# JJKK1313/DiTreeOnlinePlanner

Hardware: AMD Instinct MI355X
Metric: candidate tree-expansions/sec (carmaze, H=32) (higher is better)
Workload: dtype f16x3; 1 GPU; cfgs/carmaze.yaml + fm_policy flow sampler (K=1), batch=1024 candidates per GPU, H=32 (4 chunks x 8 steps), boxes.csv 20x20, 1024-node tree snapshot, seeded random weights; batch_per_gpu=1024, global_batch=1024, edge_length=32, action_horizon=8, pred_horizon=64, flow_steps=1, tree_nodes=1024, parallelism=candidates sharded x1

## Files before the change

ditreeonlineplanner_amd/csrc/denoise.h:

```cpp
#pragma once
#include <hip/hip_runtime.h>
#include <stdint.h>

enum { MODE_BIAS = 0, MODE_GN_MISH = 1, MODE_GN_MISH_FILM = 2, MODE_GN_MISH_RES = 3 };

enum { ST_BF16 = 0, ST_F32 = 1, ST_F16 = 2 };
static inline int fmt_make(int st, bool split) { return st | (split ? 4 : 0); }
static inline __host__ __device__ int fmt_st(int f) { return f & 3; }
static inline __host__ __device__ bool fmt_split(int f) { return (f & 4) != 0; }
static inline int fmt_es(int f) { return fmt_st(f) == ST_F32 ? 4 : 2; }

struct ConvGemmParams {
  const void* A;
  int lda;
  int in_Lp;
  int in_stride;
  int in_off;
  int taps, Cin;
  const void* W;
  void* Out;
  int ldc;
  int out_Lp, out_stride, out_off;
  int out_coff;
  int L;
  int M, N;
  const float* bias;
  int mode;
  const float* gamma;
  const float* beta;
  int group_ch;
  float eps;
  const float* film;
  int film_ld, film_off;
  const void* Res;
  int ldres, res_Lp, res_off;
  int out_f32;
  int dbg;
  int c2d, c2_H, c2_W, c2_OW, c2_OHW, c2_stride, c2_pad;
  signed char c2_kh[12], c2_kw[12];
  const void* zero;
  long long a_plane, w_plane, out_plane, res_plane;
  float w_scale;
  int splitk;
  long long slab_stride;
  float* sk_ws;
  int* sk_cnt;
  int* sat;
};

void denoise_set_dry_run(bool on);
void launch_conv_gemm(const ConvGemmParams& p, int fmt, hipStream_t s);
bool conv2d_small_eligible(int fmt);
int conv_gemm_kind(const ConvGemmParams& p, int fmt);
bool conv_gemm_supported(const ConvGemmParams& p, int fmt);
void launch_prep_sample(const float* x, void* A0, int B, int P, int D, int fmt, long long plane, hipStream_t s, int* sat = nullptr);
void launch_time_embed(float t, const float* W1, const float* b1, const float* W2, const float* b2, float* out,
                       hipStream_t s);
void launch_prep_cond(const float* temb, const float* map_emb, int E, int E_ld, const float* cond, int G, void* out, int B,
                      int Kpad, int fmt, long long plane, hipStream_t s, int* sat = nullptr);
struct FlowStep {
  int mode;
  float dt;
  float sb, sa, c0, c1, sigma;
  const float* z;
  long long z_row;
  const int* z_idx;
  int z_row0;
};
void launch_final_proj_flow(const void* Y, int C, int Lp, long long plane, const float* W, const float* bias, int D, float* x,
                            FlowStep fs, const double* act_norm , double* actions, int B, int P, int fmt,
                            hipStream_t s);
struct TapList {
  int n;
  signed char kh[49], kw[49];
};
void launch_gn1d(void* x, int ld, int Lp, int row_off, int coff, int L, int C, const float* gamma, const float* beta, float eps,
                 int mode, const float* film, int film_ld, int film_off, const void* res, int ldres, int res_Lp, int res_off,
                 int B, int fmt, long long x_plane, long long res_plane, hipStream_t s, int* sat = nullptr);
void launch_encoder_stem(const float* lm, int n, const float* W, const float* gamma, const float* beta, void* out, int B, float eps,
                         int fmt, long long plane, hipStream_t s, int* sat = nullptr);
void launch_im2col2d(const void* in, bool src_f32, void* out, int B, int H, int W, int C, const TapList& taps, int stride,
                     int pad, int OH, int OW, int Kpad, int fmt, hipStream_t s);
void launch_gn2d(const float* in, int nslab, long long slab_stride, const float* gamma, const float* beta, const void* res,
                 int relu, void* out, int B, int HW, int C, float eps, int fmt, long long res_plane, long long out_plane,
                 hipStream_t s, int* sat = nullptr);
void launch_maxpool2d(const void* in, void* out, int B, int H, int W, int C, int OH, int OW, int fmt, hipStream_t s);
void launch_avgpool2d(const void* in, void* out, int B, int HW, int C, int fmt, long long in_plane, long long out_plane,
                      hipStream_t s);
void launch_unpack_act(const void* in, int ld, int coff, int Lp, int roff, float* out, int B, int L, int C, int fmt,
                       long long plane, hipStream_t s);
```

ditreeonlineplanner_amd/csrc/denoise_host.hip:

```cpp
#include <algorithm>
#include <cmath>
#include <cstring>
#include <functional>
#include <map>
#include <sstream>
#include <thread>

#include "denoise.h"
#include "ditree_internal.h"

namespace {

struct HostParam {
  std::vector<int64_t> dims;
  const float* data = nullptr;
  int64_t n = 0;
};

struct Act {
  void* p = nullptr;
  int L = 0, C = 0;
  int ld = 0, coff = 0;
  bool padded = true;
  long long plane = 0;
// ... 321 lines not shown
    p.Out = (void*)aptr(out); p.ldc = out.ld; p.out_Lp = out.Lp(); p.out_stride = 1; p.out_off = 1; p.out_coff = 0;
    p.L = in.L; p.N = Cout; p.bias = vec(wname + ".bias"); p.mode = mode; p.eps = 1e-5f;
    if (mode >= MODE_GN_MISH) {
      p.gamma = vec(gn + ".weight"); p.beta = vec(gn + ".bias"); p.group_ch = Cout / 8;
    }
    if (mode == MODE_GN_MISH_FILM) { p.film = film; p.film_ld = film_cols; p.film_off = film_off; }
    if (mode == MODE_GN_MISH_RES) {
      p.Res = aptr(*res); p.ldres = res->ld; p.res_Lp = res->Lp(); p.res_off = res->padded ? 1 : 0; p.res_plane = res->plane;
    }
    emit_block(ops, p, out, in.L);
  }
  void emit_block(std::vector<std::function<void(int, int, hipStream_t)>>& ops, const ConvGemmParams& p, const Act& out, int L) {
    const int Cout = p.N, mode = p.mode, uf = ufmt;
    const int gch = Cout / 8;
    static const bool short_unfused = [] { const char* e = getenv("DITREE_GN_SHORT_UNFUSED"); return e && atoi(e) != 0; }();
    const bool short_fusable = (L == 8 || L == 4) && fmt_st(uf) != ST_F32 && !short_unfused;
    const bool fused = mode < MODE_GN_MISH ||
                       ((Cout & 255) == 0 && (gch == 64 || gch == 128 || gch == 256) && ((L & 15) == 0 || short_fusable));
    const bool fused_needs_tiles = fused && mode >= MODE_GN_MISH && (L & 15) != 0;
    ConvGemmParams qf = p, q = p;
    q.mode = MODE_BIAS;
    const float* film_p = p.film;
    const int film_ld_ = p.film_ld, film_off_ = p.film_off, ldres = p.ldres, res_Lp = p.res_Lp, res_off = p.res_off;
    const void* resp = p.Res;
    const float *ga = p.gamma, *be = p.beta;
    void* xo = (void*)out.p;
    const int ld = out.ld, oLp = out.Lp(), ocoff = out.coff;
    const long long xpl = out.plane, rpl = p.res_plane;
    int* gsat = p.sat;
    ops.push_back([=, this](int, int Bp, hipStream_t s) mutable {
      if (fused && (!fused_needs_tiles || ((Bp * L) & 255) == 0)) {
        qf.M = Bp * L;
        run_gemm(qf, uf, s);
        return;
      }
      q.M = Bp * L;
      run_gemm(q, uf, s);
      note_other();
      launch_gn1d(xo, ld, oLp, 1, ocoff, L, Cout, ga, be, 1e-5f, mode, film_p, film_ld_, film_off_, resp, ldres, res_Lp,
                  res_off, Bp, uf, xpl, rpl, s, gsat);
    });
  }
  void add_conv1(std::vector<std::function<void(int, int, hipStream_t)>>& ops, const std::string& wname, const Act& in,
                 const Act& out) {
    const HostParam& w = P_(wname + ".weight");
    const int Cout = (int)w.dims[0], Cin = (int)w.dims[1];
    const float* wd = w.data;
    const Packed wp = pack(wname, ufmt, Cout, 1, Cin, [=](int n, int, int ci) { return wd[(size_t)n * Cin + ci]; });
    ConvGemmParams p{};
    p.A = aptr(in); p.lda = in.ld; p.in_Lp = in.Lp(); p.in_stride = 1; p.in_off = 1; p.taps = 1; p.Cin = Cin;
    set_w(p, wp); set_in(p, in); set_out(p, out);
    p.sat = sat_slot(wname, ufmt);
    p.Out = (void*)aptr(out); p.ldc = out.ld; p.out_Lp = out.Lp(); p.out_stride = 1; p.out_off = 1;
    p.L = in.L; p.N = Cout; p.bias = vec(wname + ".bias"); p.mode = MODE_BIAS;
    const int L = in.L, uf = ufmt;
    ops.push_back([this, p, L, uf](int, int Bp, hipStream_t s) mutable {
      p.M = Bp * L;
      run_gemm(p, uf, s);
    });
  }
  void add_down(std::vector<std::function<void(int, int, hipStream_t)>>& ops, const std::string& wname, const Act& in,
                const Act& out) {
    const HostParam& w = P_(wname + ".weight");
    const int Cout = (int)w.dims[0], Cin = (int)w.dims[1];
    const float* wd = w.data;
    const Packed wp = pack(wname, ufmt, Cout, 3, Cin, [=](int n, int t, int ci) { return wd[((size_t)n * Cin + ci) * 3 + t]; });
    ConvGemmParams p{};
    p.A = aptr(in); p.lda = in.ld; p.in_Lp = in.Lp(); p.in_stride = 2; p.in_off = 0; p.taps = 3; p.Cin = Cin;
    set_w(p, wp); set_in(p, in); set_out(p, out);
    p.sat = sat_slot(wname, ufmt);
    p.Out = (void*)aptr(out); p.ldc = out.ld; p.out_Lp = out.Lp(); p.out_stride = 1; p.out_off = 1;
    p.L = out.L; p.N = Cout; p.bias = vec(wname + ".bias"); p.mode = MODE_BIAS;
    const int L = out.L, uf = ufmt;
    ops.push_back([this, p, L, uf](int, int Bp, hipStream_t s) mutable {
      p.M = Bp * L;
      run_gemm(p, uf, s);
    });
  }
  void add_up(std::vector<std::function<void(int, int, hipStream_t)>>& ops, const std::string& wname, const Act& in,
              const Act& out) {
    const HostParam& w = P_(wname + ".weight");
    const int Cin = (int)w.dims[0], Cout = (int)w.dims[1];
    const float* wd = w.data;
    for (int par = 0; par < 2; ++par) {
      const int k0 = par == 0 ? 3 : 2, k1 = par == 0 ? 1 : 0;
      const Packed wp = pack(wname + (par ? ".odd" : ".even"), ufmt, Cout, 2, Cin, [=](int n, int t, int ci) {
        return wd[((size_t)ci * Cout + n) * 4 + (t == 0 ? k0 : k1)];
      });
      ConvGemmParams p{};
      p.A = aptr(in); p.lda = in.ld; p.in_Lp = in.Lp(); p.in_stride = 1; p.in_off = par; p.taps = 2; p.Cin = Cin;
      set_w(p, wp); set_in(p, in); set_out(p, out);
      p.sat = sat_slot(wname, ufmt);
      p.Out = (void*)aptr(out); p.ldc = out.ld; p.out_Lp = out.Lp(); p.out_stride = 2; p.out_off = 1 + par;
      p.L = in.L; p.N = Cout; p.bias = vec(wname + ".bias"); p.mode = MODE_BIAS;
      const int L = in.L, uf = ufmt;
      ops.push_back([this, p, L, uf](int, int Bp, hipStream_t s) mutable {
        p.M = Bp * L;
        run_gemm(p, uf, s);
      });
    }
  }

  void add_crb(const std::string& pre, const Act& in, const Act& out, int& film_cursor, const std::string& tag) {
    const int Cout = (int)P_(pre + ".blocks.0.block.0.weight").dims[0];
    Act h = make_act(tag + ".h", in.L, Cout);
    const int film_off = film_cursor;
    film_cursor += 2 * Cout;
    add_conv3(unet_ops, pre + ".blocks.0.block.0", in, h, MODE_GN_MISH_FILM, pre + ".blocks.0.block.1", film_off, nullptr);
    Act res = in;
    if (has(pre + ".residual_conv.weight")) {
      res = make_act(tag + ".res", in.L, Cout);
      add_conv1(unet_ops, pre + ".residual_conv", in, res);
    }
    add_conv3(unet_ops, pre + ".blocks.1.block.0", h, out, MODE_GN_MISH_RES, pre + ".blocks.1.block.1", 0, &res);
  }

  void build(int prec_, int Bmax_);
};

void DenoiserState::build(int prec_, int Bmax_) {
  free_workspace();
  prec = prec_;
  switch (prec) {
    case DITREE_PREC_BF16: ufmt = fmt_make(ST_BF16, false); efmt = ST_BF16; break;
    case DITREE_PREC_F32: ufmt = fmt_make(ST_F32, false); efmt = ST_F32; break;
    case DITREE_PREC_F16X3: ufmt = fmt_make(ST_F16, true); efmt = ufmt; break;
    case DITREE_PREC_BF16X3: ufmt = fmt_make(ST_BF16, true); efmt = ufmt; break;
    case DITREE_PREC_F16: ufmt = fmt_make(ST_F16, false); efmt = ST_F16; break;
    default: throw std::runtime_error("unknown precision");
  }
  sat_flags = (int*)dalloc(SAT_SLOTS * sizeof(int));
  sat_cond = sat_slot("cond_encoder input: Mish(time | map embedding | observation)", ufmt);
  sat_sample = sat_slot("sample (the noisy action sequence)", ufmt);
  const int C0 = dims[0], C1 = dims[1], C2 = dims[2];
  const int L0 = P, L1 = P / 2, L2 = P / 4;
  if (P % 16 != 0 || P < 16 || P > 256 || (256 % P) != 0) throw std::runtime_error("pred_horizon must be 16, 32, 64, 128 or 256");
  bgran = fmt_st(ufmt) != ST_F32 ? std::max(16, 1024 / P) : 16;
  Buser = Bmax_;
  Bmax = (Bmax_ + bgran - 1) / bgran * bgran;
  {
    const long long per_sample = std::max({(long long)(L2 + 2) * 2 * C2, (long long)(L1 + 2) * 2 * C1, (long long)(L0 + 2) * C0,
                                           (long long)L0 * 64}) * fmt_es(ufmt);
    long long cap = std::min<long long>(8192, 0x7f000000LL / per_sample);
    cap = cap / 256 * 256;
    if (cap < 256) throw std::runtime_error("denoiser too large for one 256-sample work unit");
    if (Bmax > cap) Bmax = (int)cap;
  }
  if (fmt_split(ufmt) && ((C0 | C1 | C2) & 255) != 0)
    throw std::runtime_error("the split precisions need down_dims that are multiples of 256 (halo / gemm16 tiles)");
  x_cur = (float*)dalloc((size_t)Bmax * P * D * 4);
  temb = (float*)dalloc(256 * 4);
  condK = (cond_dim + 63) / 64 * 64;
  const int Brows = (Bmax + 255) / 256 * 256;
  E_ld = fmt_split(efmt) ? (E + 255) / 256 * 256 : E;
  map_emb = (float*)dalloc((size_t)Brows * E_ld * 4);
  cond_plane = planes() == 2 ? (long long)Brows * condK * es() : 0;
  condA = dalloc((size_t)Brows * condK * es() * planes());

  std::vector<std::string> crbs = {"unet.down_modules.0.0", "unet.down_modules.0.1", "unet.down_modules.1.0",
                                   "unet.down_modules.1.1", "unet.down_modules.2.0", "unet.down_modules.2.1",
                                   "unet.mid_modules.0",    "unet.mid_modules.1",    "unet.up_modules.0.0",
                                   "unet.up_modules.0.1",   "unet.up_modules.1.0",   "unet.up_modules.1.1"};
  film_cols = 0;
  std::vector<int> film_offs;
  for (auto& c : crbs) {
    film_offs.push_back(film_cols);
// ... 782 lines not shown
```

ditreeonlineplanner_amd/csrc/denoise_kernels.hip:

```cpp
#include <cstdlib>
#include <type_traits>

#include <stdexcept>

#include "denoise.h"

static thread_local bool g_dn_dry_run = false;
void denoise_set_dry_run(bool on) { g_dn_dry_run = on; }
#define DN_LAUNCH(...) do { if (!g_dn_dry_run) hipLaunchKernelGGL(__VA_ARGS__); } while (0)

typedef __attribute__((ext_vector_type(8))) __bf16 bf16x8_t;
typedef __attribute__((ext_vector_type(8))) _Float16 half8_t;
typedef __attribute__((ext_vector_type(8))) short short8_t;
typedef __attribute__((ext_vector_type(4))) short short4_t;
typedef __attribute__((ext_vector_type(16))) float f32x16_t;
typedef __attribute__((ext_vector_type(4))) float f32x4_t;
typedef __attribute__((ext_vector_type(2))) float f32x2_t;
typedef __attribute__((ext_vector_type(2))) _Float16 half2_t;
typedef __attribute__((ext_vector_type(2))) short short2_t;

#define GLOBAL_AS __attribute__((address_space(1)))
#define LDS_AS __attribute__((address_space(3)))

__device__ __forceinline__ unsigned short f2bf(float f) {
// ... 450 lines not shown
#pragma unroll
      for (int i = 0; i < 16; ++i) acc[mb][j][i] = 0.0f;

  const int swl = (r5 >> 1) & 7;
  const int a_row_off = (wm * 64 + r5) * 128;
  const int b_row_off = 32768 + (wn * 128 + r5) * 128;

  auto kstep = [&](const char* sb, auto stage_tag, char* snext) {
    constexpr bool STAGE = decltype(stage_tag)::value;
    if constexpr (PREC != 1) {
      short8_t af[2][2], bfr[2][4];
      auto rd = [&](int ks, int slot) {
        const int ps = (((ks << 1) | h) ^ swl) << 4;
#pragma unroll
        for (int mb = 0; mb < 2; ++mb)
          af[slot][mb] = *(const short8_t*)(sb + a_row_off + mb * 4096 + ps);
#pragma unroll
        for (int j = 0; j < 4; ++j)
          bfr[slot][j] = *(const short8_t*)(sb + b_row_off + j * 4096 + ps);
      };
      if constexpr (STAGE) {
#pragma unroll
        for (int q = 0; q < 8; ++q) stage_piece(q, snext);
      }
      rd(0, 0);
#pragma unroll
      for (int ks = 0; ks < 4; ++ks) {
        if (ks < 3) rd(ks + 1, (ks + 1) & 1);
#pragma unroll
        for (int mb = 0; mb < 2; ++mb)
#pragma unroll
          for (int j = 0; j < 4; ++j)
            acc[mb][j] = mfma32<ET>(af[ks & 1][mb], bfr[ks & 1][j], acc[mb][j]);
      }
      if constexpr (STAGE) __builtin_amdgcn_sched_group_barrier(0x020, 8, 0);
      __builtin_amdgcn_sched_group_barrier(0x100, 6, 0);
#pragma unroll
      for (int ks = 0; ks < 4; ++ks) {
        if (ks < 3) __builtin_amdgcn_sched_group_barrier(0x100, 6, 0);
        __builtin_amdgcn_sched_group_barrier(0x008, 8, 0);
      }
    } else {
#pragma unroll
      for (int sl = 0; sl < 8; ++sl) {
        const int ps = (sl ^ swl) << 4;
        f32x4_t af[2], bfr[4];
#pragma unroll
        for (int mb = 0; mb < 2; ++mb) af[mb] = *(const f32x4_t*)(sb + a_row_off + mb * 4096 + ps);
#pragma unroll
        for (int j = 0; j < 4; ++j) bfr[j] = *(const f32x4_t*)(sb + b_row_off + j * 4096 + ps);
#pragma unroll
        for (int s2 = 0; s2 < 2; ++s2) {
#pragma unroll
          for (int mb = 0; mb < 2; ++mb) {
            const float a = h ? af[mb][2 * s2 + 1] : af[mb][2 * s2];
#pragma unroll
            for (int j = 0; j < 4; ++j) {
              const float bv = h ? bfr[j][2 * s2 + 1] : bfr[j][2 * s2];
              acc[mb][j] = __builtin_amdgcn_mfma_f32_32x32x2f32(a, bv, acc[mb][j], 0, 0, 0);
            }
          }
        }
        if constexpr (STAGE) stage_piece(sl, snext);
      }
    }
  };

#pragma unroll
  for (int q = 0; q < 8; ++q) stage_piece(q, smem);
  advance();
  for (int kt = 0; kt < nk - 1; ++kt) {
    asm volatile("s_waitcnt vmcnt(0)" ::: "memory");
    __syncthreads();
    kstep(smem + (kt & 1) * 65536, std::true_type{}, smem + ((kt + 1) & 1) * 65536);
    advance();
  }
  asm volatile("s_waitcnt vmcnt(0)" ::: "memory");
  __syncthreads();
  kstep(smem + ((nk - 1) & 1) * 65536, std::false_type{}, nullptr);
  __syncthreads();
  gemm_epilogue<PREC>(p, acc, smem, tm, tn, tid, lane, r5, h, wm, wn, out_extra);
}

template <int ET, bool SPLIT, bool SHORT = false>
__device__ __forceinline__ void gemm_epilogue16(const ConvGemmParams& p, f32x4_t (&acc)[4][8], char* smem, int tm, int tn,
                                                int tid, int lane, int r4, int h4, int wm, int wn) {
  const int c_l = wn * 128 + 8 * r4;
  const int n0 = tn * 256 + c_l;
  {
    f32x4_t b0 = {0.f, 0.f, 0.f, 0.f}, b1 = b0;
    if (p.bias != nullptr) { b0 = *(const f32x4_t*)(p.bias + n0); b1 = *(const f32x4_t*)(p.bias + n0 + 4); }
    if constexpr (ET == 1) {
      const float ws = p.w_scale;
#pragma unroll
      for (int mb = 0; mb < 4; ++mb)
#pragma unroll
        for (int j = 0; j < 4; ++j) { acc[mb][j] = acc[mb][j] * ws + b0[j]; acc[mb][4 + j] = acc[mb][4 + j] * ws + b1[j]; }
    } else if (p.bias != nullptr) {
#pragma unroll
      for (int mb = 0; mb < 4; ++mb)
#pragma unroll
        for (int j = 0; j < 4; ++j) { acc[mb][j] += b0[j]; acc[mb][4 + j] += b1[j]; }
    }
  }
  constexpr bool short_l = SHORT;
  const int lane_b = short_l ? (4 * h4) / p.L : 0, lane_l = -lane_b * p.L;
  int blk_b[4], blk_l[4];
#pragma unroll
  for (int mb = 0; mb < 4; ++mb) {
    const int m0 = tm * 256 + wm * 64 + mb * 16;
    const int b = m0 / p.L;
    blk_b[mb] = b;
    blk_l[mb] = m0 - b * p.L;
  }
  auto store_row = [&](char* o, const float (&v)[8]) {
    short8_t hi, lo;
    if constexpr (ET == 1) {
      sat_check_row(p.sat, v);
#pragma unroll
      for (int jj = 0; jj < 4; ++jj) {
        const f32x2_t c = {__builtin_amdgcn_fmed3f(v[2 * jj], -65504.0f, 65504.0f),
                           __builtin_amdgcn_fmed3f(v[2 * jj + 1], -65504.0f, 65504.0f)};
        const half2_t h = __builtin_convertvector(c, half2_t);
        const short2_t hs = __builtin_bit_cast(short2_t, h);
        hi[2 * jj] = hs[0]; hi[2 * jj + 1] = hs[1];
        if constexpr (SPLIT) {
          const half2_t l = __builtin_convertvector(c - __builtin_convertvector(h, f32x2_t), half2_t);
          const short2_t ls = __builtin_bit_cast(short2_t, l);
          lo[2 * jj] = ls[0]; lo[2 * jj + 1] = ls[1];
        }
      }
    } else {
#pragma unroll
      for (int j = 0; j < 8; ++j) {
        hi[j] = (short)f2bf(v[j]);
        if constexpr (SPLIT) lo[j] = (short)f2bf(v[j] - bf2f((unsigned short)hi[j]));
      }
    }
    *(short8_t*)o = hi;
    if constexpr (SPLIT) *(short8_t*)(o + p.out_plane) = lo;
  };
  auto out_ptr = [&](int mb, int esize) {
    const long long orow = (long long)(blk_b[mb] + lane_b) * p.out_Lp + (long long)(blk_l[mb] + 4 * h4 + lane_l) * p.out_stride + p.out_off;
    return (char*)p.Out + (orow * p.ldc + p.out_coff + n0) * esize;
  };
  if (p.mode < MODE_GN_MISH) {
    const int esize = p.out_f32 ? 4 : 2;
    const long long ostep = (long long)p.out_stride * p.ldc * esize;
#pragma unroll
    for (int mb = 0; mb < 4; ++mb) {
      char* ob = out_ptr(mb, esize);
#pragma unroll
      for (int i = 0; i < 4; ++i, ob += ostep) {
        float v[8];
#pragma unroll
        for (int j = 0; j < 8; ++j) v[j] = acc[mb][j][i];
        if (p.out_f32) {
          *(f32x4_t*)ob = f32x4_t{v[0], v[1], v[2], v[3]};
          *(f32x4_t*)(ob + 16) = f32x4_t{v[4], v[5], v[6], v[7]};
        } else {
          store_row(ob, v);
        }
      }
    }
    return;
  }
  const bool has_film = p.mode == MODE_GN_MISH_FILM, has_res = p.mode == MODE_GN_MISH_RES;
  const int spt = 256 / p.L;
  const int ns = spt > 16 ? spt * 4 : 64;
  float* s_sum = (float*)smem;
  float* s_sq = s_sum + ns;
  float* s_gb = s_sq + ns;
  float* s_film = s_gb + 512;
  const bool film_direct = has_film && short_l;
  const int b_last = p.M / p.L - 1;
  for (int i = tid; i < 2 * ns; i += 512) s_sum[i] = 0.0f;
  s_gb[tid] = tid < 256 ? p.gamma[tn * 256 + tid] : p.beta[tn * 256 + tid - 256];
  if (has_film && !film_direct) {
    for (int idx = tid; idx < spt * 128; idx += 512) {
      const int sm = idx >> 7, c4 = idx & 127;
      const int b = min(tm * spt + sm, b_last);
      const float* src = p.film + (long long)b * p.film_ld + p.film_off + tn * 256 + (c4 & 63) * 4 + (c4 >> 6) * p.N;
      *(f32x4_t*)(s_film + sm * 512 + c4 * 4) = *(const f32x4_t*)src;
    }
  }
  f32x4_t rh[2], rl[2];
  const long long rstep = (long long)p.ldres * 2;
  auto fetch_film = [&](int mb) {
    const float* fr = p.film + (long long)min(blk_b[mb] + lane_b, b_last) * p.film_ld + p.film_off + n0;
    rh[0] = *(const f32x4_t*)fr; rh[1] = *(const f32x4_t*)(fr + 4);
    rl[0] = *(const f32x4_t*)(fr + p.N); rl[1] = *(const f32x4_t*)(fr + p.N + 4);
  };
  if (film_direct) fetch_film(0);
  auto fetch_res = [&](int r) {
    const long long rrow = (long long)(blk_b[r >> 2] + lane_b) * p.res_Lp + blk_l[r >> 2] + 4 * h4 + lane_l + p.res_off;
    const char* rp = (const char*)p.Res + (rrow * p.ldres + n0) * 2 + (r & 3) * rstep;
    rh[r & 1] = *(const f32x4_t*)rp;
    if constexpr (SPLIT) rl[r & 1] = *(const f32x4_t*)(rp + p.res_plane);
  };
  if (has_res) { fetch_res(0); fetch_res(1); }
  __syncthreads();
  const int gi = c_l / p.group_ch;
  const bool wide = p.group_ch >= 128;
  const float inv_cnt = 1.0f / (float)(p.group_ch * p.L);
  int slot[4];
#pragma unroll
  for (int mb = 0; mb < 4; ++mb) slot[mb] = (blk_b[mb] + lane_b - tm * spt) * 4 + gi;
  const int hsame = short_l ? (p.L == 8 ? 2 : 1) : 4;
  const bool adder = (r4 == 0 || (!wide && r4 == 8)) && (h4 & (hsame - 1)) == 0;
  auto block_sums = [&](float (&s)[4], float* cell) {
#pragma unroll
    for (int mb = 0; mb < 4; ++mb) s[mb] = dpp_add<0xB1>(s[mb]);
#pragma unroll
    for (int mb = 0; mb < 4; ++mb) s[mb] = dpp_add<0x4E>(s[mb]);
#pragma unroll
    for (int mb = 0; mb < 4; ++mb) s[mb] = dpp_add<0x141>(s[mb]);
    if (wide) {
#pragma unroll
      for (int mb = 0; mb < 4; ++mb) s[mb] = dpp_add<0x140>(s[mb]);
    }
    if (hsame >= 2) {
#pragma unroll
      for (int mb = 0; mb < 4; ++mb) s[mb] += __shfl_xor(s[mb], 16);
    }
    if (hsame == 4) {
#pragma unroll
      for (int mb = 0; mb < 4; ++mb) s[mb] += __shfl_xor(s[mb], 32);
    }
    if (adder) {
#pragma unroll
      for (int mb = 0; mb < 4; ++mb) atomicAdd(&cell[slot[mb]], s[mb]);
    }
  };
  float mean_[4], rstd_[4];
  auto pair = [&](int mb, int j, int ip) { return f32x2_t{acc[mb][j][2 * ip], acc[mb][j][2 * ip + 1]}; };
  if constexpr (!SPLIT) {
    float s[4], q[4];
#pragma unroll
    for (int mb = 0; mb < 4; ++mb) {
      f32x2_t s2 = {0.f, 0.f}, q2 = {0.f, 0.f};
#pragma unroll
      for (int j = 0; j < 8; ++j)
#pragma unroll
        for (int ip = 0; ip < 2; ++ip) {
          const f32x2_t v = pair(mb, j, ip);
          s2 += v;
          q2 = __builtin_elementwise_fma(v, v, q2);
        }
      s[mb] = s2[0] + s2[1];
// ... 905 lines not shown
      mm16(0, 0, 0);
      __builtin_amdgcn_sched_group_barrier(0x100, 4, 0);
      __builtin_amdgcn_sched_group_barrier(0x008, 16, 0);
      __builtin_amdgcn_sched_barrier(0);
      mm16(1, 0, 0);
      __builtin_amdgcn_sched_barrier(0);
      mm16(0, 1, 1);
      __builtin_amdgcn_sched_barrier(0);
    } else {
      rdB(1, k, 0, 1);
      mm16(0, 0, 0);
      __builtin_amdgcn_sched_group_barrier(0x100, 4, 0);
      __builtin_amdgcn_sched_group_barrier(0x008, 16, 0);
      __builtin_amdgcn_sched_barrier(0);
      rdA(1, k, 1);
      rdB(0, k, 1, 0);
      mm16(0, 1, 1);
      __builtin_amdgcn_sched_group_barrier(0x100, 8, 0);
      __builtin_amdgcn_sched_group_barrier(0x008, 16, 0);
      __builtin_amdgcn_sched_barrier(0);
      rdB(1, k, 1, 1);
      mm16(1, 0, 0);
      __builtin_amdgcn_sched_group_barrier(0x100, 4, 0);
      __builtin_amdgcn_sched_group_barrier(0x008, 16, 0);
      __builtin_amdgcn_sched_barrier(0);
    }
    int ao2 = 0, wo2 = 0;
    if constexpr (ISSUE) src_off(k + 2, ao2, wo2);
    if constexpr (HAS_NEXT) {
      asm volatile("s_waitcnt vmcnt(0) lgkmcnt(0)" ::: "memory");
      __builtin_amdgcn_s_barrier();
      rdA(0, k + 1, 0);
      rdB(0, k + 1, SPLIT ? 1 : 0, 0);
    }
#pragma unroll
    for (int mb = 0; mb < 4; ++mb)
#pragma unroll
      for (int jj = 0; jj < 4; ++jj) {
        mm(1, 1, 1, mb, (mb & 1) ? 3 - jj : jj);
        if constexpr (ISSUE) {
          const int m = mb * 4 + jj, i = (m & 1) ? -1 : (m >> 1);
          if (i >= 0 && i < 4)
            __builtin_amdgcn_raw_ptr_buffer_load_lds(a_rsrc, (LDS_AS void*)(smem + (k & 1) * BUF + (w * 4 + i) * 1024), 16,
                                                     (i & 1) ? pao : pae, aq[i] + ao2, 0, 0);
          else if (!SPLIT && i >= 4 && i < 8)
            __builtin_amdgcn_raw_ptr_buffer_load_lds(w_rsrc, (LDS_AS void*)(smem + W_BASE + (k & 1) * BUF + (w * 4 + i - 4) * 1024),
                                                     16, ((i - 4) & 1) ? pbo : pbe, wq[i - 4] + wo2, 0, 0);
        }
      }
    if constexpr (HAS_NEXT) __builtin_amdgcn_sched_group_barrier(0x100, 8, 1);
#pragma unroll
    for (int i = 0; i < 16; ++i) {
      __builtin_amdgcn_sched_group_barrier(0x008, 1, 1);
      if (ISSUE && !(i & 1) && (!SPLIT || i < 8)) __builtin_amdgcn_sched_group_barrier(0x020, 1, 1);
    }
    __builtin_amdgcn_sched_barrier(0);
  };
  using Tt = std::true_type;
  using Ff = std::false_type;

  issue(0);
  asm volatile("s_waitcnt vmcnt(0)" ::: "memory");
  __builtin_amdgcn_s_barrier();
  if (nk > 1) {
    if constexpr (SPLIT) {
      int ao, wo;
      src_off(1, ao, wo);
#pragma unroll
      for (int q = 0; q < 4; ++q)
        __builtin_amdgcn_raw_ptr_buffer_load_lds(a_rsrc, (LDS_AS void*)(smem + BUF + (w * 4 + q) * 1024), 16, (q & 1) ? pao : pae,
                                                 aq[q] + ao, 0, 0);
    } else {
      issue(1);
    }
  }
  rdA(0, 0, 0);
  rdB(0, 0, SPLIT ? 1 : 0, 0);
  for (int k = 0; k < nk - 2; ++k) step(Tt{}, Tt{}, k);
  if (nk >= 2) step(Tt{}, Ff{}, nk - 2);
  step(Ff{}, Ff{}, nk - 1);
  __syncthreads();
  gemm_epilogue16<ET, SPLIT, SHORT>(p, acc, smem, tm, tn, tid, lane, r4, h4, wm, wn);
}
static bool gemm16_eligible(const ConvGemmParams& p, int fmt) {
  const bool short_ok = p.L == 8 || p.L == 4;
  return fmt_st(fmt) != ST_F32 && !p.c2d && (!p.out_f32 || p.mode == MODE_BIAS) && p.taps >= 1 && p.taps <= 3 && (p.M & 255) == 0 &&
         (p.N & 255) == 0 && (p.Cin & 63) == 0 && ((p.L & 15) == 0 || short_ok) && p.M > 0 &&
         (p.mode == MODE_BIAS || (256 % p.L) == 0);
}
static bool halo_eligible(const ConvGemmParams& p, int fmt) {
  static const bool l8_off = [] { const char* e = getenv("DITREE_HALO_L8"); return e && atoi(e) == 0; }();
  static const bool l4_off = [] { const char* e = getenv("DITREE_HALO_L4"); return e && atoi(e) == 0; }();
  const bool l_ok = p.L >= 16 || (p.L == 8 && fmt_split(fmt) && !l8_off) || (p.L == 4 && fmt_split(fmt) && !l4_off && p.splitk <= 1);
  return fmt_st(fmt) != ST_F32 && !p.c2d && p.taps == 3 && p.in_stride == 1 && p.in_Lp == p.L + 2 && (256 % p.L) == 0 &&
         l_ok && (p.M & 255) == 0 && (p.N & 255) == 0 && (p.Cin & 63) == 0 && p.Cin >= 192;
}
bool conv2d_small_eligible(int fmt) { return fmt_st(fmt) != ST_F32; }
int conv_gemm_kind(const ConvGemmParams& p, int fmt) { return halo_eligible(p, fmt) ? 0 : (p.c2d ? 2 : 1); }
bool conv_gemm_supported(const ConvGemmParams& p, int fmt) {
  return !fmt_split(fmt) || halo_eligible(p, fmt) || gemm16_eligible(p, fmt) ||
         (p.c2d && (p.N & 63) == 0 && (p.Cin & 63) == 0 && p.out_f32 && p.mode == MODE_BIAS);
}

static void ensure_lds_attrs() {
  static bool done[64] = {};
  int dev = 0;
  hipGetDevice(&dev);
  if (dev < 0 || dev >= 64 || done[dev]) return;
  done[dev] = true;
  const hipFuncAttribute at = hipFuncAttributeMaxDynamicSharedMemorySize;
  hipFuncSetAttribute((const void*)conv_gemm_kernel<0, false>, at, 131072);
  hipFuncSetAttribute((const void*)conv_gemm_kernel<1, false>, at, 131072);
  hipFuncSetAttribute((const void*)conv_gemm_kernel<2, false>, at, 131072);
  hipFuncSetAttribute((const void*)conv_gemm_kernel<0, true>, at, 131072);
  hipFuncSetAttribute((const void*)conv_gemm_kernel<1, true>, at, 131072);
  hipFuncSetAttribute((const void*)conv_gemm_kernel<2, true>, at, 131072);
  hipFuncSetAttribute((const void*)conv3_halo16_kernel<0, false>, at, 147456);
  hipFuncSetAttribute((const void*)conv3_halo16_kernel<1, false>, at, 147456);
  hipFuncSetAttribute((const void*)conv3_halo16x3_kernel<0>, at, 147456);
  hipFuncSetAttribute((const void*)conv3_halo16x3_kernel<1>, at, 147456);
  hipFuncSetAttribute((const void*)conv3_halo16x3_kernel<0, true>, at, 147456);
  hipFuncSetAttribute((const void*)conv3_halo16x3_kernel<1, true>, at, 147456);
  hipFuncSetAttribute((const void*)conv3_halo16x3_kernel<0, false, true>, at, 147456);
  hipFuncSetAttribute((const void*)conv3_halo16x3_kernel<1, false, true>, at, 147456);
  hipFuncSetAttribute((const void*)conv3_halo16x3_kernel<0, true, true>, at, 147456);
  hipFuncSetAttribute((const void*)conv3_halo16x3_kernel<1, true, true>, at, 147456);
  hipFuncSetAttribute((const void*)conv3_halo16x3_kernel<0, true, false, 6>, at, 163840);
  hipFuncSetAttribute((const void*)conv3_halo16x3_kernel<1, true, false, 6>, at, 163840);
  hipFuncSetAttribute((const void*)gemm16_kernel<0, false>, at, 131072);
  hipFuncSetAttribute((const void*)gemm16_kernel<1, false>, at, 131072);
  hipFuncSetAttribute((const void*)gemm16_kernel<0, true>, at, 131072);
  hipFuncSetAttribute((const void*)gemm16_kernel<1, true>, at, 131072);
  hipFuncSetAttribute((const void*)gemm16_kernel<0, false, true>, at, 131072);
  hipFuncSetAttribute((const void*)gemm16_kernel<1, false, true>, at, 131072);
  hipFuncSetAttribute((const void*)gemm16_kernel<0, true, true>, at, 131072);
  hipFuncSetAttribute((const void*)gemm16_kernel<1, true, true>, at, 131072);
}

void launch_conv_gemm(const ConvGemmParams& p, int fmt, hipStream_t s) {
  ensure_lds_attrs();
  const int st = fmt_st(fmt);
  const bool split = fmt_split(fmt), f16 = st == ST_F16;
  const int ntn = (p.N + 255) >> 8, ntm = (p.M + 255) >> 8;
  const dim3 grid(ntm * ntn), block(512);
  if (halo_eligible(p, fmt)) {
    if (split && p.splitk > 1) {
      if (p.sk_ws == nullptr || p.sk_cnt == nullptr || ((p.Cin >> 5) % p.splitk) != 0 || (p.Cin >> 5) / p.splitk < 2)
        throw std::runtime_error("conv_gemm: split-K of the halo kernel needs its workspace and splitk | Cin / 32, >= 2 chunks each");
      const dim3 gsk(ntm * ntn, p.splitk);
      if (p.L == 8) {
        if (f16) DN_LAUNCH((conv3_halo16x3_kernel<1, true, true>), gsk, block, 147456, s, p);
        else DN_LAUNCH((conv3_halo16x3_kernel<0, true, true>), gsk, block, 147456, s, p);
      } else if (f16) DN_LAUNCH((conv3_halo16x3_kernel<1, false, true>), gsk, block, 147456, s, p);
      else DN_LAUNCH((conv3_halo16x3_kernel<0, false, true>), gsk, block, 147456, s, p);
      return;
    }
    if (split && p.L == 4) {
      if (f16) DN_LAUNCH((conv3_halo16x3_kernel<1, true, false, 6>), grid, block, 163840, s, p);
      else DN_LAUNCH((conv3_halo16x3_kernel<0, true, false, 6>), grid, block, 163840, s, p);
      return;
    }
    if (split) {
      if (p.L == 8) {
        if (f16) DN_LAUNCH((conv3_halo16x3_kernel<1, true>), grid, block, 147456, s, p);
        else DN_LAUNCH((conv3_halo16x3_kernel<0, true>), grid, block, 147456, s, p);
      } else if (f16) DN_LAUNCH(conv3_halo16x3_kernel<1>, grid, block, 147456, s, p);
      else DN_LAUNCH(conv3_halo16x3_kernel<0>, grid, block, 147456, s, p);
    } else {
      if (f16) DN_LAUNCH((conv3_halo16_kernel<1, false>), grid, block, 147456, s, p);
      else DN_LAUNCH((conv3_halo16_kernel<0, false>), grid, block, 147456, s, p);
    }
    return;
  }
  if (gemm16_eligible(p, fmt) && (p.L & 15) != 0) {
    if (split) {
      if (f16) DN_LAUNCH((gemm16_kernel<1, true, true>), grid, block, 131072, s, p);
      else DN_LAUNCH((gemm16_kernel<0, true, true>), grid, block, 131072, s, p);
    } else {
      if (f16) DN_LAUNCH((gemm16_kernel<1, false, true>), grid, block, 131072, s, p);
      else DN_LAUNCH((gemm16_kernel<0, false, true>), grid, block, 131072, s, p);
    }
    return;
  }
  if (gemm16_eligible(p, fmt)) {
    if (split) {
      if (f16) DN_LAUNCH((gemm16_kernel<1, true>), grid, block, 131072, s, p);
      else DN_LAUNCH((gemm16_kernel<0, true>), grid, block, 131072, s, p);
    } else {
      if (f16) DN_LAUNCH((gemm16_kernel<1, false>), grid, block, 131072, s, p);
      else DN_LAUNCH((gemm16_kernel<0, false>), grid, block, 131072, s, p);
    }
    return;
  }
  if (p.mode >= MODE_GN_MISH && (p.L & 15) != 0)
    throw std::runtime_error("conv_gemm: a fused GroupNorm epilogue at L = 8 / 4 exists on the gemm16 tile only (whole 256-row tiles)");
  if (p.c2d && conv2d_small_eligible(fmt) && (p.N & 63) == 0 && (p.Cin & 63) == 0 && p.out_f32 && p.mode == MODE_BIAS) {
    const dim3 g2(((p.M + 63) >> 6) * (p.N >> 6), p.splitk > 1 ? p.splitk : 1);
    if (split) {
      if (f16) DN_LAUNCH((conv2d_small_kernel<1, true>), g2, dim3(256), 3 * 16384, s, p);
      else DN_LAUNCH((conv2d_small_kernel<0, true>), g2, dim3(256), 3 * 16384, s, p);
    } else {
      if (f16) DN_LAUNCH((conv2d_small_kernel<1, false>), g2, dim3(256), 3 * 16384, s, p);
      else DN_LAUNCH((conv2d_small_kernel<0, false>), g2, dim3(256), 3 * 16384, s, p);
    }
    return;
  }
  if (split) throw std::runtime_error("conv_gemm: a split GEMM of this shape fits no tile (conv_gemm_supported is the contract)");
  if (p.c2d) {
    const dim3 grid2(ntm * ntn, p.splitk > 1 ? p.splitk : 1);
    if (st == ST_F32) DN_LAUNCH((conv_gemm_kernel<1, true>), grid2, block, 131072, s, p);
    else if (f16) DN_LAUNCH((conv_gemm_kernel<2, true>), grid2, block, 131072, s, p);
    else DN_LAUNCH((conv_gemm_kernel<0, true>), grid2, block, 131072, s, p);
    return;
  }
  if (st == ST_F32) DN_LAUNCH((conv_gemm_kernel<1, false>), grid, block, 131072, s, p);
  else if (f16) DN_LAUNCH((conv_gemm_kernel<2, false>), grid, block, 131072, s, p);
  else DN_LAUNCH((conv_gemm_kernel<0, false>), grid, block, 131072, s, p);
}

template <int FMT>
__device__ __forceinline__ void store_elem(void* base, long long idx, float v, long long plane = 0) {
  constexpr int ST = FMT & 3;
  if constexpr (ST == ST_F32) {
    ((float*)base)[idx] = v;
  } else {
    constexpr int ET = ST == ST_F16 ? 1 : 0;
    const unsigned short hi = f2e<ET>(v);
// ... 676 lines not shown
```

Baseline: 19410 candidate expansions/s.

## Merge even/odd transposed-conv GEMMs into one halo-loaded up2 kernel

The stride-2 transposed convolution (upsample) used to run as two separate GEMM launches, one per output parity, each reading the same input. It now packs both parities' weights into one N=2*Cout matrix and runs a new gemm16_up2_kernel. That kernel loads the padded input rows once into LDS and reads the two taps as shifted rows, with the epilogue interleaving the outputs by parity. This saves a launch and a second input read per upsample, but adds a large hand-scheduled kernel with a bias-only epilogue and an env-var fallback.

```diff
diff --git a/ditreeonlineplanner_amd/csrc/denoise.h b/ditreeonlineplanner_amd/csrc/denoise.h
--- a/ditreeonlineplanner_amd/csrc/denoise.h
+++ b/ditreeonlineplanner_amd/csrc/denoise.h
@@ -46,6 +46,7 @@
   float* sk_ws;
   int* sk_cnt;
   int* sat;
+  int up2;
 };
 
 void denoise_set_dry_run(bool on);
diff --git a/ditreeonlineplanner_amd/csrc/denoise_host.hip b/ditreeonlineplanner_amd/csrc/denoise_host.hip
--- a/ditreeonlineplanner_amd/csrc/denoise_host.hip
+++ b/ditreeonlineplanner_amd/csrc/denoise_host.hip
@@ -427,6 +427,27 @@
     const HostParam& w = P_(wname + ".weight");
     const int Cin = (int)w.dims[0], Cout = (int)w.dims[1];
     const float* wd = w.data;
+    const char* old_walk = getenv("DITREE_GEMM16_OLD_WALK");
+    if (fmt_split(ufmt) && !(old_walk && atoi(old_walk) != 0) && (Cout & 127) == 0 && (in.L & 15) == 0 && (256 % in.L) == 0 &&
+        (Cin & 63) == 0) {
+      const Packed wp = pack(wname + ".up2", ufmt, 2 * Cout, 2, Cin, [=](int n, int t, int ci) {
+        const int par = (n >> 7) & 1, co = (n >> 8) * 128 + (n & 127);
+        const int k = par == 0 ? (t == 0 ? 3 : 1) : (t == 0 ? 2 : 0);
+        return wd[((size_t)ci * Cout + co) * 4 + k];
+      });
+      ConvGemmParams p{};
+      p.A = aptr(in); p.lda = in.ld; p.in_Lp = in.Lp(); p.in_stride = 1; p.in_off = 0; p.taps = 2; p.Cin = Cin;
+      set_w(p, wp); set_in(p, in); set_out(p, out);
+      p.sat = sat_slot(wname, ufmt);
+      p.Out = (void*)aptr(out); p.ldc = out.ld; p.out_Lp = out.Lp(); p.out_stride = 2; p.out_off = 1;
+      p.L = in.L; p.N = 2 * Cout; p.bias = vec(wname + ".bias"); p.mode = MODE_BIAS; p.up2 = 1;
+      const int L = in.L, uf = ufmt;
+      ops.push_back([this, p, L, uf](int, int Bp, hipStream_t s) mutable {
+        p.M = Bp * L;
+        run_gemm(p, uf, s);
+      });
+      return;
+    }
     for (int par = 0; par < 2; ++par) {
       const int k0 = par == 0 ? 3 : 2, k1 = par == 0 ? 1 : 0;
       const Packed wp = pack(wname + (par ? ".odd" : ".even"), ufmt, Cout, 2, Cin, [=](int n, int t, int ci) {
diff --git a/ditreeonlineplanner_amd/csrc/denoise_kernels.hip b/ditreeonlineplanner_amd/csrc/denoise_kernels.hip
--- a/ditreeonlineplanner_amd/csrc/denoise_kernels.hip
+++ b/ditreeonlineplanner_amd/csrc/denoise_kernels.hip
@@ -556,11 +556,11 @@
   gemm_epilogue<PREC>(p, acc, smem, tm, tn, tid, lane, r5, h, wm, wn, out_extra);
 }
 
-template <int ET, bool SPLIT, bool SHORT = false>
+template <int ET, bool SPLIT, bool SHORT = false, bool UP2 = false>
 __device__ __forceinline__ void gemm_epilogue16(const ConvGemmParams& p, f32x4_t (&acc)[4][8], char* smem, int tm, int tn,
                                                 int tid, int lane, int r4, int h4, int wm, int wn) {
   const int c_l = wn * 128 + 8 * r4;
-  const int n0 = tn * 256 + c_l;
+  const int n0 = UP2 ? tn * 128 + 8 * r4 : tn * 256 + c_l;
   {
     f32x4_t b0 = {0.f, 0.f, 0.f, 0.f}, b1 = b0;
     if (p.bias != nullptr) { b0 = *(const f32x4_t*)(p.bias + n0); b1 = *(const f32x4_t*)(p.bias + n0 + 4); }
@@ -615,7 +615,8 @@
     if constexpr (SPLIT) *(short8_t*)(o + p.out_plane) = lo;
   };
   auto out_ptr = [&](int mb, int esize) {
-    const long long orow = (long long)(blk_b[mb] + lane_b) * p.out_Lp + (long long)(blk_l[mb] + 4 * h4 + lane_l) * p.out_stride + p.out_off;
+    const long long orow = (long long)(blk_b[mb] + lane_b) * p.out_Lp + (long long)(blk_l[mb] + 4 * h4 + lane_l) * p.out_stride + p.out_off +
+                           (UP2 ? wn : 0);
     return (char*)p.Out + (orow * p.ldc + p.out_coff + n0) * esize;
   };
   if (p.mode < MODE_GN_MISH) {
@@ -639,6 +640,7 @@
     }
     return;
   }
+  if constexpr (UP2) return;
   const bool has_film = p.mode == MODE_GN_MISH_FILM, has_res = p.mode == MODE_GN_MISH_RES;
   const int spt = 256 / p.L;
   const int ns = spt > 16 ? spt * 4 : 64;
@@ -1710,22 +1712,228 @@
   __syncthreads();
   gemm_epilogue16<ET, SPLIT, SHORT>(p, acc, smem, tm, tn, tid, lane, r4, h4, wm, wn);
 }
+
+template <int ET>
+__global__ void __launch_bounds__(512, 2) gemm16_up2_kernel(ConvGemmParams p) {
+  extern __shared__ __attribute__((aligned(16))) char smem[];
+  constexpr int NP = 5;
+  constexpr int A_BUF = NP * 8192, W_BUF = 32768, W_BASE = 2 * A_BUF;
+  const int tid = threadIdx.x, lane = tid & 63;
+  const int w = __builtin_amdgcn_readfirstlane(tid >> 6);
+  const int r4 = lane & 15, h4 = lane >> 4;
+  const int wm = w >> 1, wn = w & 1;
+  const int ntn = p.N >> 8, ntm = p.M >> 8;
+  const int tile = xcd_remap_strips(blockIdx.x, ntm, ntn, p.dbg);
+  const int tm = tile / ntn, tn = tile - tm * ntn;
+  const int L = p.L, Lp = p.in_Lp, S = 256 / L;
+  const int a_rows = S * Lp;
+  const int nv = p.Cin >> 5;
+  const long long K = 2LL * p.Cin;
+  const unsigned a_plane = (unsigned)p.a_plane, w_plane = (unsigned)p.w_plane;
+
+  unsigned pa0, pa4, pbe;
+  const char* const a_base = (const char*)p.A + ((long long)tm * S * Lp + p.in_off) * p.lda * 2;
+  const char* const w_base = (const char*)p.W + ((long long)tn * 256) * K * 2;
+  const __amdgpu_buffer_rsrc_t a_rsrc = __builtin_amdgcn_make_buffer_rsrc((void*)a_base, 0, 0x7fffffff, 0x00020000);
+  const __amdgpu_buffer_rsrc_t w_rsrc = __builtin_amdgcn_make_buffer_rsrc((void*)w_base, 0, 0x7fffffff, 0x00020000);
+  {
+    const int r = w * 8 + (lane >> 3);
+    const int slot = (lane & 7) ^ (r & 7);
+    const unsigned po = (slot & 4) ? a_plane : 0u;
+    pa0 = (unsigned)((r * p.lda + (slot & 3) * 8) * 2) + po;
+    const int r4r = r + 256;
+    const int rs = r4r < a_rows ? r4r : a_rows - 1;
+    pa4 = (unsigned)((rs * p.lda + (slot & 3) * 8) * 2) + po;
+  }
+  const int a_piece = 64 * p.lda * 2;
+  int wq[4];
+  {
+    const int lr = lane >> 3;
+    const int slot0 = (lane & 7) ^ lr;
+    pbe = (unsigned)(((long long)(8 * lr) * K + (slot0 & 3) * 8) * 2) + ((slot0 & 4) ? w_plane : 0u);
+#pragma unroll
+    for (int q = 0; q < 4; ++q) {
+      const int r0 = (w * 4 + q) * 8;
+      const int cu = (r0 & 128) + 8 * (r0 & 8) + ((r0 >> 4) & 7);
+      wq[q] = (int)((long long)cu * K * 2);
+    }
+  }
+  const int w_tap = p.Cin * 2;
+  auto issue_a = [&](int v, int i) {
+    __builtin_amdgcn_raw_ptr_buffer_load_lds(a_rsrc, (LDS_AS void*)(smem + (v & 1) * A_BUF + (w + 8 * i) * 1024), 16,
+                                             i < 4 ? pa0 : pa4, v * 64 + (i < 4 ? i * a_piece : 0), 0, 0);
+  };
+  auto issue_w = [&](int v, int t, int q) {
+    __builtin_amdgcn_raw_ptr_buffer_load_lds(w_rsrc, (LDS_AS void*)(smem + W_BASE + t * W_BUF + (w * 4 + q) * 1024), 16, pbe,
+                                             wq[q] + v * 64 + t * w_tap, 0, 0);
+  };
+
+  int lrow0;
+  {
+    const int ml = wm * 64 + r4;
+    const int sb = ml / L;
+    lrow0 = sb * Lp + (ml - sb * L) + wn;
+  }
+  int lstep[4];
+#pragma unroll
+  for (int mb = 0; mb < 4; ++mb) lstep[mb] = 16 * mb + 2 * (((wm * 64 + 16 * mb) / L) - ((wm * 64) / L));
+  const int swl = r4 & 7;
+  const int b_row_off = (wn * 128 + r4) * 128;
+
+  f32x4_t acc[4][8];
+#pragma unroll
+  for (int mb = 0; mb < 4; ++mb)
+#pragma unroll
+    for (int j = 0; j < 8; ++j) acc[mb][j] = f32x4_t{0.f, 0.f, 0.f, 0.f};
+
+  short8_t af[2][4], bq[2][4];
+  auto rdA = [&](int set, int v, int t, int pl) {
+    const char* ab = smem + (v & 1) * A_BUF;
+#pragma unroll
+    for (int mb = 0; mb < 4; ++mb) {
+      const int row = lrow0 + lstep[mb] + t;
+      const int ps = (((pl << 2) | h4) ^ (row & 7)) << 4;
+      af[set][mb] = *(const short8_t*)(ab + row * 128 + ps);
+    }
+  };
+  auto rdB = [&](int set, int t, int pl, int half) {
+    const char* wb = smem + W_BASE + t * W_BUF + b_row_off + half * 8192;
+    const int psb = (((pl << 2) | h4) ^ swl) << 4;
+#pragma unroll
+    for (int jj = 0; jj < 4; ++jj) bq[set][jj] = *(const short8_t*)(wb + jj * 2048 + psb);
+  };
+  auto mm = [&](int aset, int bset, int half, int mb, int jj) {
+    acc[mb][half * 4 + jj] = mfma16<ET>(af[aset][mb], bq[bset][jj], acc[mb][half * 4 + jj]);
+  };
+  auto mm16 = [&](int aset, int bset, int half) {
+#pragma unroll
+    for (int mb = 0; mb < 4; ++mb)
+#pragma unroll
+      for (int jj = 0; jj < 4; ++jj) mm(aset, bset, half, mb, (mb & 1) ? 3 - jj : jj);
+  };
+  auto step = [&](auto tT, auto tNext, auto tIW, auto tIA, auto tVM, int v) {
+    constexpr int T = decltype(tT)::value;
+    constexpr bool HAS_NEXT = decltype(tNext)::value, ISSUE_W = decltype(tIW)::value, ISSUE_A = decltype(tIA)::value;
+    constexpr int VM = decltype(tVM)::value;
+    asm volatile("" : "+v"(lrow0));
+    __builtin_amdgcn_s_setprio(2);
+    rdB(1, T, 1, 1);
+    mm16(0, 0, 0);
+    __builtin_amdgcn_sched_group_barrier(0x100, 4, 0);
+    __builtin_amdgcn_sched_group_barrier(0x008, 16, 0);
+    __builtin_amdgcn_sched_barrier(0);
+    rdB(0, T, 0, 0);
+    rdA(1, v, T, 1);
+    mm16(0, 1, 1);
+    __builtin_amdgcn_sched_group_barrier(0x100, 8, 0);
+    __builtin_amdgcn_sched_group_barrier(0x008, 16, 0);
+    __builtin_amdgcn_sched_barrier(0);
+    __builtin_amdgcn_s_setprio(1);
+    rdB(1, T, 0, 1);
+    mm16(0, 0, 0);
+    __builtin_amdgcn_sched_group_barrier(0x100, 4, 0);
+    __builtin_amdgcn_sched_group_barrier(0x008, 16, 0);
+    __builtin_amdgcn_sched_barrier(0);
+    mm16(1, 0, 0);
+    if constexpr (ISSUE_A) {
+      if constexpr (T == 0) { issue_a(v + 1, 0); issue_a(v + 1, 1); issue_a(v + 1, 2); }
+      else { issue_a(v + 1, 3); issue_a(v + 1, 4); }
+      __builtin_amdgcn_sched_group_barrier(0x008, 4, 2);
+      __builtin_amdgcn_sched_group_barrier(0x020, 1, 2);
+      __builtin_amdgcn_sched_group_barrier(0x008, 4, 2);
+      __builtin_amdgcn_sched_group_barrier(0x020, 1, 2);
+      __builtin_amdgcn_sched_group_barrier(0x008, 4, 2);
+      if constexpr (T == 0) __builtin_amdgcn_sched_group_barrier(0x020, 1, 2);
+      __builtin_amdgcn_sched_group_barrier(0x008, 4, 2);
+    }
+    __builtin_amdgcn_sched_barrier(0);
+    __builtin_amdgcn_s_setprio(0);
+    mm16(0, 1, 1);
+    __builtin_amdgcn_sched_barrier(0);
+    if constexpr (HAS_NEXT) {
+      if constexpr (VM == 0) asm volatile("s_waitcnt vmcnt(0) lgkmcnt(0)" ::: "memory");
+      else asm volatile("s_waitcnt vmcnt(3) lgkmcnt(0)" ::: "memory");
+      __builtin_amdgcn_s_barrier();
+      __builtin_amdgcn_s_setprio(3);
+      constexpr int T1 = T ^ 1;
+      rdA(0, v + T, T1, 0);
+      rdB(0, T1, 1, 0);
+    }
+#pragma unroll
+    for (int mb = 0; mb < 4; ++mb)
+#pragma unroll
+      for (int jj = 0; jj < 4; ++jj) {
+        mm(1, 1, 1, mb, (mb & 1) ? 3 - jj : jj);
+        const int i = mb * 4 + jj;
+        const int d = (i & 1) ? -1 : (i >> 1);
+        if constexpr (ISSUE_W) { if (d >= 0 && d < 4) issue_w(v + 1, T, d); }
+      }
+    if constexpr (HAS_NEXT) __builtin_amdgcn_sched_group_barrier(0x100, 8, 1);
+    constexpr int NV = ISSUE_W ? 4 : 0;
+#pragma unroll
+    for (int i = 0; i < 16; ++i) {
+      __builtin_amdgcn_sched_group_barrier(0x008, 1, 1);
+      if (!(i & 1) && (i >> 1) < NV) __builtin_amdgcn_sched_group_barrier(0x020, 1, 1);
+    }
+    __builtin_amdgcn_sched_barrier(0);
+  };
+  using I0 = std::integral_constant<int, 0>;
+  using I1 = std::integral_constant<int, 1>;
+  using I3 = std::integral_constant<int, 3>;
+  using Tt = std::true_type;
+  using Ff = std::false_type;
+
+#pragma unroll
+  for (int i = 0; i < NP; ++i) issue_a(0, i);
+#pragma unroll
+  for (int q = 0; q < 4; ++q) issue_w(0, 0, q);
+  asm volatile("s_waitcnt vmcnt(0)" ::: "memory");
+  __builtin_amdgcn_s_barrier();
+#pragma unroll
+  for (int q = 0; q < 4; ++q) issue_w(0, 1, q);
+  rdA(0, 0, 0, 0);
+  rdB(0, 0, 1, 0);
+  for (int v = 0; v < nv - 2; ++v) {
+    step(I0{}, Tt{}, Tt{}, Tt{}, I3{}, v);
+    step(I1{}, Tt{}, Tt{}, Tt{}, I0{}, v);
+  }
+  {
+    const int v = nv - 2;
+    step(I0{}, Tt{}, Tt{}, Tt{}, I0{}, v);
+    step(I1{}, Tt{}, Tt{}, Tt{}, I0{}, v);
+  }
+  {
+    const int v = nv - 1;
+    step(I0{}, Tt{}, Ff{}, Ff{}, I0{}, v);
+    step(I1{}, Ff{}, Ff{}, Ff{}, I0{}, v);
+  }
+  __builtin_amdgcn_s_setprio(0);
+  __syncthreads();
+  gemm_epilogue16<ET, true, false, true>(p, acc, smem, tm, tn, tid, lane, r4, h4, wm, wn);
+}
+
 static bool gemm16_eligible(const ConvGemmParams& p, int fmt) {
   const bool short_ok = p.L == 8 || p.L == 4;
   return fmt_st(fmt) != ST_F32 && !p.c2d && (!p.out_f32 || p.mode == MODE_BIAS) && p.taps >= 1 && p.taps <= 3 && (p.M & 255) == 0 &&
          (p.N & 255) == 0 && (p.Cin & 63) == 0 && ((p.L & 15) == 0 || short_ok) && p.M > 0 &&
          (p.mode == MODE_BIAS || (256 % p.L) == 0);
 }
+static bool up2_eligible(const ConvGemmParams& p, int fmt) {
+  return fmt_split(fmt) && fmt_st(fmt) != ST_F32 && p.up2 && !p.c2d && p.taps == 2 && p.in_stride == 1 && p.in_off == 0 &&
+         p.in_Lp == p.L + 2 && (p.L & 15) == 0 && (256 % p.L) == 0 && p.out_stride == 2 && (p.M & 255) == 0 && (p.N & 255) == 0 &&
+         (p.Cin & 63) == 0 && p.M > 0 && p.mode == MODE_BIAS && !p.out_f32 && p.splitk <= 1;
+}
 static bool halo_eligible(const ConvGemmParams& p, int fmt) {
   static const bool l8_off = [] { const char* e = getenv("DITREE_HALO_L8"); return e && atoi(e) == 0; }();
   static const bool l4_off = [] { const char* e = getenv("DITREE_HALO_L4"); return e && atoi(e) == 0; }();
   const bool l_ok = p.L >= 16 || (p.L == 8 && fmt_split(fmt) && !l8_off) || (p.L == 4 && fmt_split(fmt) && !l4_off && p.splitk <= 1);
-  return fmt_st(fmt) != ST_F32 && !p.c2d && p.taps == 3 && p.in_stride == 1 && p.in_Lp == p.L + 2 && (256 % p.L) == 0 &&
+  return fmt_st(fmt) != ST_F32 && !p.up2 && !p.c2d && p.taps == 3 && p.in_stride == 1 && p.in_Lp == p.L + 2 && (256 % p.L) == 0 &&
          l_ok && (p.M & 255) == 0 && (p.N & 255) == 0 && (p.Cin & 63) == 0 && p.Cin >= 192;
 }
 bool conv2d_small_eligible(int fmt) { return fmt_st(fmt) != ST_F32; }
 int conv_gemm_kind(const ConvGemmParams& p, int fmt) { return halo_eligible(p, fmt) ? 0 : (p.c2d ? 2 : 1); }
 bool conv_gemm_supported(const ConvGemmParams& p, int fmt) {
+  if (p.up2) return up2_eligible(p, fmt);
   return !fmt_split(fmt) || halo_eligible(p, fmt) || gemm16_eligible(p, fmt) ||
          (p.c2d && (p.N & 63) == 0 && (p.Cin & 63) == 0 && p.out_f32 && p.mode == MODE_BIAS);
 }
@@ -1755,6 +1963,8 @@
   hipFuncSetAttribute((const void*)conv3_halo16x3_kernel<1, true, true>, at, 147456);
   hipFuncSetAttribute((const void*)conv3_halo16x3_kernel<0, true, false, 6>, at, 163840);
   hipFuncSetAttribute((const void*)conv3_halo16x3_kernel<1, true, false, 6>, at, 163840);
+  hipFuncSetAttribute((const void*)gemm16_up2_kernel<0>, at, 147456);
+  hipFuncSetAttribute((const void*)gemm16_up2_kernel<1>, at, 147456);
   hipFuncSetAttribute((const void*)gemm16_kernel<0, false>, at, 131072);
   hipFuncSetAttribute((const void*)gemm16_kernel<1, false>, at, 131072);
   hipFuncSetAttribute((const void*)gemm16_kernel<0, true>, at, 131072);
@@ -1771,6 +1981,12 @@
   const bool split = fmt_split(fmt), f16 = st == ST_F16;
   const int ntn = (p.N + 255) >> 8, ntm = (p.M + 255) >> 8;
   const dim3 grid(ntm * ntn), block(512);
+  if (p.up2) {
+    if (!up2_eligible(p, fmt)) throw std::runtime_error("conv_gemm: a merged transposed conv runs on gemm16_up2_kernel only");
+    if (f16) DN_LAUNCH(gemm16_up2_kernel<1>, grid, block, 147456, s, p);
+    else DN_LAUNCH(gemm16_up2_kernel<0>, grid, block, 147456, s, p);
+    return;
+  }
   if (halo_eligible(p, fmt)) {
     if (split && p.splitk > 1) {
       if (p.sk_ws == nullptr || p.sk_cnt == nullptr || ((p.Cin >> 5) % p.splitk) != 0 || (p.Cin >> 5) / p.splitk < 2)
```

Measured after the change: 19440 candidate expansions/s, median of 6. Within noise of the previous version (+0.2%).
